# sleep3r/crispy

Hardware: NVIDIA B200
Metric: stream-seconds of 48 kHz audio denoised per wall-second (higher is better)
Workload: dtype f32

## Files before the change

### crispy_b200/csrc/ns_pipe.cuh

```cuda
#pragma once
#include "ns_common.h"
#include "ns_simt.h"

namespace ns {

NS_DEV f4 ld4(const float *p) { return *reinterpret_cast<const f4 *>(p); }

constexpr int kHpThreads = 96;
#ifndef NS_HP_TILE
#define NS_HP_TILE 96
#endif
constexpr int kHpTile = NS_HP_TILE;
constexpr int kHpPitch = kHpTile + 4;
constexpr int kHpStages = 4;
constexpr int kHpAhead = 2;
constexpr int kHpRaw16 = (2 * kHpTile - 8 + 15) / 16 * 16;
static_assert(kFrame % kHpTile == 0 && kHpTile % 8 == 0 && kHpPitch % 32 != 0 && kHpPitch % 4 == 0, "tile geometry");
static_assert(kHpRaw16 % 16 == 0 && kHpRaw16 + 2 * kHpTile <= kHpPitch * 4 && 2 * kHpTile - 8 <= kHpRaw16, "PCM16 staging");
struct HpSmem {
  float tile[kHpStages][32][kHpPitch];
  int landed[kHpStages], done[kHpStages], freed[kHpStages];
};

NS_DEV float load_sample(const Params &p, int stream, long long idx) {
// ... 168 lines not shown
        float v[kHist / 32];
#pragma unroll
        for (int i = 0; i < kHist / 32; i++) v[i] = src[lane + 32 * i];
#pragma unroll
        for (int i = 0; i < kHist / 32; i++) dst[lane + 32 * i] = v[i];
      }
    }
  }
}

#ifndef NS_HP_PAR
#define NS_HP_PAR 1
#endif
constexpr int kHpSeg = 4;
constexpr int kHpSegLen = kHpTile / kHpSeg;
constexpr int kHpYStages = 2;
constexpr int kHpParThreads = 256;
constexpr int kHpParAhead = 1;
static_assert(kHpTile % (4 * kHpSeg) == 0, "segments are whole 16-byte groups");
#ifdef NS_HOST_EMU
inline long long g_hp_respeculated = 0;
#define NS_HP_COUNT_RESPEC() __atomic_add_fetch(&::ns::g_hp_respeculated, 1, __ATOMIC_RELAXED)
#else
#define NS_HP_COUNT_RESPEC() ((void)0)
#endif
#if defined(NS_HP_CLOCKS) && defined(__CUDACC__) && !defined(NS_HOST_EMU)
#define NS_HP_T0() const long long hp_t0_ = clock64()
#define NS_HP_ACC(var) var += clock64() - hp_t0_
#else
#define NS_HP_T0() ((void)0)
#define NS_HP_ACC(var) ((void)0)
#endif
struct HpParSmem {
  HpSmem x;
  float y[kHpYStages][32][kHpPitch];
  float spec[2][kHpSeg + 1][32][2];
  float exact[2][kHpSeg][32][2];
  alignas(16) int bad[2][32][kHpSeg];
  int go;
  int ver;
  int ydone;
  int yfreed;
};

NS_DEV float hp_fast_err(float a, float b, float s) {
  const float ea = b - (s - a), eb = a - (s - b);
  return fabsf(a) >= fabsf(b) ? ea : eb;
}

NS_DEV void highpass_par_body(const Params &p, HpParSmem &sm) {
  const int tid = Simt::tid();
  const int lane = tid & 31, warp = tid >> 5;
  const int s0 = Simt::cta() * 32;
  const int nrows = (p.n_streams - s0) < 32 ? (p.n_streams - s0) : 32;
  const int nsamp = p.n_frames * kFrame;
  const int ntiles = nsamp / kHpTile;
  const bool tail_direct = nsamp >= kHist;
  if (tid < kHpStages) sm.x.landed[tid] = sm.x.done[tid] = sm.x.freed[tid] = 0;
  if (tid == 0) sm.ver = sm.go = sm.ydone = sm.yfreed = 0;
  Simt::cta_sync();
  const long long in0 = (long long)p.frame0 * kFrame;
  const bool in16 = (p.flags & kFlagInI16) != 0;
  const int amask = in16 ? 7 : 3;
  const bool fast = (p.in_stride & amask) == 0 && (in0 & amask) == 0 && (reinterpret_cast<uintptr_t>(p.in) & 15) == 0;
  const bool raw16 = fast && in16;
  const float scale = ((p.flags & kFlagUnitScale) && !in16) ? 32768.0f : 1.0f;
  const bool valid = lane < nrows;
  float m0 = 0.f, m1 = 0.f;
  long long t_work = 0, t_wait = 0, t_wait2 = 0;
  (void)t_work, (void)t_wait, (void)t_wait2;
  const long long t_begin = 0;
  (void)t_begin;
  const double na0 = -(double)-1.99599f, na1 = -(double)0.99600f;
  auto exact_run = [&](const float *xrow, float *yrow, int n4) {
#pragma unroll 2
    for (int c = 0; c < 4 * n4; c += 4) {
      const f4 xv = ld4(xrow + c);
      const float x[4] = {xv.x * scale, xv.y * scale, xv.z * scale, xv.w * scale};
      float y[4];
#pragma unroll
      for (int i = 0; i < 4; i++) {
        const float xi = x[i];
        const float yi = xi + m0;
        const double xd = (double)xi, yd = (double)yi;
        m0 = (float)((double)m1 + fma(na0, yd, -2.0 * xd));
        m1 = (float)fma(na1, yd, xd);
        y[i] = yi;
      }
      *reinterpret_cast<f4 *>(yrow + c) = f4{y[0], y[1], y[2], y[3]};
    }
  };
  if (warp == 1) {
    for (int n = 0; n < ntiles + kHpParAhead; n++) {
      if (n < ntiles) {
        if (n >= kHpStages) {
          NS_HP_T0();
          Simt::flag_wait(&sm.x.freed[n % kHpStages], n - kHpStages + 1, true);
          NS_HP_ACC(t_wait);
        }
        hp_fetch_tile(p, sm.x, s0, nrows, in0, n, fast, lane);
      }
      Simt::cp_async_commit();
      if (n >= kHpParAhead) {
        Simt::cp_async_wait<kHpParAhead>();
        if (raw16) {
          Simt::warp_sync();
          if (lane < nrows) {
            float *row = sm.x.tile[(n - kHpParAhead) % kHpStages][lane];
#pragma unroll 4
            for (int c = 0; c < kHpTile; c += 4) {
              const uint32_t *rw = reinterpret_cast<const uint32_t *>(reinterpret_cast<const char *>(row) + kHpRaw16 + 2 * c);
              const uint32_t r0 = rw[0], r1 = rw[1];
              *reinterpret_cast<f4 *>(row + c) = f4{(float)(int16_t)(r0 & 0xFFFFu), (float)(int16_t)(r0 >> 16),
                                                    (float)(int16_t)(r1 & 0xFFFFu), (float)(int16_t)(r1 >> 16)};
            }
          }
        }
        Simt::fence_cta();
        Simt::warp_sync();
        if (lane == 0) Simt::flag_set(&sm.x.landed[(n - kHpParAhead) % kHpStages], n - kHpParAhead + 1);
      }
    }
  } else if (warp == 0) {
    float *st = p.state + (long long)(s0 + (valid ? lane : 0)) * kStateFloats;
    if (valid) m0 = st[kStHp], m1 = st[kStHp + 1];
    const float a0f = 1.99599f, na1f = -0.99600f;
    auto spec_tile = [&](int n) {
      const float *row = sm.x.tile[n % kHpStages][lane];
      float(*rec)[32][2] = sm.spec[n & 1];
      for (int v = 0; v < kHpSeg; v++) {
        rec[v][lane][0] = m0, rec[v][lane][1] = m1;
#pragma unroll 2
        for (int c = v * kHpSegLen; c < (v + 1) * kHpSegLen; c += 4) {
          const f4 xv = ld4(row + c);
          const float x[4] = {xv.x * scale, xv.y * scale, xv.z * scale, xv.w * scale};
#pragma unroll
          for (int i = 0; i < 4; i++) {
            const float xi = x[i];
            const float yi = xi + m0;
            const float ph = a0f * yi, pl = fmaf(a0f, yi, -ph);
            const float b = -2.0f * xi;
            const float ch = fmaf(-2.0f, xi, m1), cl = hp_fast_err(m1, b, ch);
            const float s1 = ch + ph;
            const float e1 = hp_fast_err(ch, ph, s1);
            m0 = s1 + ((cl + pl) + e1);
            m1 = fmaf(na1f, yi, xi);
          }
        }
      }
      rec[kHpSeg][lane][0] = m0, rec[kHpSeg][lane][1] = m1;
    };
    auto settle = [&](int k, bool next_speculated) {
      Simt::flag_poll(&sm.ver, kHpSeg * (k + 1), false);
      Simt::fence_cta();
      if (valid) {
        static_assert(kHpSeg == 4, "one 16-byte load fetches a lane's four flags");
        struct alignas(16) I4 {
          int x, y, z, w;
        };
        const I4 bd = *reinterpret_cast<const I4 *>(sm.bad[k & 1][lane]);
        const int v0 = bd.x ? 0 : bd.y ? 1 : bd.z ? 2 : bd.w ? 3 : -1;
        if (v0 >= 0) {
          NS_HP_COUNT_RESPEC();
          m0 = sm.exact[k & 1][v0][lane][0], m1 = sm.exact[k & 1][v0][lane][1];
          const int c0 = (v0 + 1) * kHpSegLen;
          exact_run(sm.x.tile[k % kHpStages][lane] + c0, sm.y[k % kHpYStages][lane] + c0, (kHpTile - c0) / 4);
          if (next_speculated) spec_tile(k + 1);
        }
      }
      Simt::fence_cta();
      Simt::warp_sync();
      if (lane == 0) {
        Simt::flag_store(&sm.ydone, k + 1);
        Simt::flag_store(&sm.x.freed[k % kHpStages], k + 1);
        if (next_speculated) Simt::flag_store(&sm.go, k + 2);
      }
    };
    for (int n = 0; n < ntiles; n++) {
      {
        NS_HP_T0();
        Simt::flag_wait(&sm.x.landed[n % kHpStages], n + 1, false);
        NS_HP_ACC(t_wait);
      }
      {
        NS_HP_T0();
        if (valid) spec_tile(n);
        NS_HP_ACC(t_work);
      }
      if (n >= 1) {
        NS_HP_T0();
        settle(n - 1, true);
        NS_HP_ACC(t_wait2);
      } else {
        Simt::fence_cta();
        Simt::warp_sync();
        if (lane == 0) Simt::flag_store(&sm.go, 1);
      }
    }
    if (ntiles > 0) settle(ntiles - 1, false);
    if (valid) {
      st[kStHp] = m0;
      st[kStHp + 1] = m1;
    }
  } else if (warp == 2) {
    hp_copy_rows(p.state + (long long)s0 * kStateFloats + kStHist, kStateFloats, p.hp + (long long)s0 * p.hp_stride,
                 p.hp_stride, nrows, lane);
    Simt::warp_sync();
    for (int n = 0; n < ntiles; n++) {
      {
        NS_HP_T0();
        Simt::flag_wait(&sm.ydone, n + 1, true);
        NS_HP_ACC(t_wait);
      }
      NS_HP_T0();
      float(*tile)[kHpPitch] = sm.y[n % kHpYStages];
      const int base = n * kHpTile;
      if (lane < kHpTile / 4) {
        const int c = 4 * lane;
        float *dsth = p.hp + (long long)s0 * p.hp_stride + kHist + base + c;
        const int hidx = base + c - (nsamp - kHist);
        if (tail_direct && hidx >= 0) {
          float *dsts = p.state + (long long)s0 * kStateFloats + kStHist + hidx;
          for (int r = 0; r < nrows; r++, dsth += p.hp_stride, dsts += kStateFloats) {
            const f4 v = ld4(&tile[r][c]);
            *reinterpret_cast<f4 *>(dsth) = v;
            *reinterpret_cast<f4 *>(dsts) = v;
          }
        } else {
#pragma unroll 8
          for (int r = 0; r < nrows; r++, dsth += p.hp_stride) *reinterpret_cast<f4 *>(dsth) = ld4(&tile[r][c]);
        }
      }
      Simt::warp_sync();
      NS_HP_ACC(t_work);
      if (lane == 0) Simt::flag_set(&sm.yfreed, n + 1);
    }
    if (!tail_direct) {
      Simt::fence_cta();
      Simt::warp_sync();
      for (int r = 0; r < nrows; r++) {
        const float *src = p.hp + (long long)(s0 + r) * p.hp_stride + nsamp;
        float *dst = p.state + (long long)(s0 + r) * kStateFloats + kStHist;
        float v[kHist / 32];
#pragma unroll
        for (int i = 0; i < kHist / 32; i++) v[i] = src[lane + 32 * i];
#pragma unroll
        for (int i = 0; i < kHist / 32; i++) dst[lane + 32 * i] = v[i];
      }
    }
  } else if (warp != 4) {
    const int v = warp == 3 ? 0 : warp - 4;
    for (int n = 0; n < ntiles; n++) {
      {
        NS_HP_T0();
        Simt::flag_wait(&sm.go, n + 1, true);
        NS_HP_ACC(t_wait);
      }
      if (n >= kHpYStages) {
        NS_HP_T0();
        Simt::flag_wait(&sm.yfreed, n - kHpYStages + 1, true);
        NS_HP_ACC(t_wait2);
      }
      NS_HP_T0();
      if (valid) {
        m0 = sm.spec[n & 1][v][lane][0], m1 = sm.spec[n & 1][v][lane][1];
        exact_run(sm.x.tile[n % kHpStages][lane] + v * kHpSegLen, sm.y[n % kHpYStages][lane] + v * kHpSegLen, kHpSegLen / 4);
        sm.exact[n & 1][v][lane][0] = m0, sm.exact[n & 1][v][lane][1] = m1;
        sm.bad[n & 1][lane][v] =
            (f2u(m0) != f2u(sm.spec[n & 1][v + 1][lane][0])) | (f2u(m1) != f2u(sm.spec[n & 1][v + 1][lane][1]));
      }
      Simt::fence_cta();
      Simt::warp_sync();
      NS_HP_ACC(t_work);
      if (lane == 0) Simt::atomic_add_shared(&sm.ver, 1);
    }
  }
#if defined(NS_HP_CLOCKS) && defined(__CUDACC__) && !defined(NS_HOST_EMU)
  if (Simt::cta() == 0 && lane == 0 && warp != 4)
    printf("K0 warp %d: %d tiles, work %lld, wait %lld, wait2 %lld cycles\n", warp, ntiles, t_work, t_wait, t_wait2);
#endif
}

template <int R>
struct PitchSmem {
  static constexpr int kHLen = R * kFrame + 1248;
  static constexpr int kXlpFloats = (R * kLpStride > kHLen) ? R * kLpStride : kHLen;
  alignas(16) float xr[R * kLpStride];
  alignas(16) float xlp[kXlpFloats];
  alignas(16) float ac[R][8];
  alignas(16) float lpc2[R][8];
  alignas(16) float fx[R][12];
  alignas(16) int fi[R][12];
  alignas(16) float xx[R];
  alignas(16) float s10[R][12];
#ifdef NS_PITCH_PAD_BYTES
  char pad[NS_PITCH_PAD_BYTES];
#endif
  int best0[R], best1[R], T0[R], nk[R];
  int n_tri[4], n_sgl[4];
  union {
    struct {
      alignas(16) float xc[R][152];
      alignas(16) float sb6[R][148];
    };
    struct {
      uint32_t tri[4][R * 16], sgl[4][R * 16];
      alignas(16) float dots[R][64];
    };
  };
};

struct Best2 {
  float n0, d0, n1, d1;
  int p0, p1;
};
NS_DEV void best_init(Best2 &b) {
  b.n0 = b.n1 = -1.f;
  b.d0 = b.d1 = 0.f;
  b.p0 = 0;
  b.p1 = 1;
}
NS_DEV void best_insert(Best2 &b, float num, float syy, int i) {
  if (num * b.d1 > b.n1 * syy) {
    if (num * b.d0 > b.n0 * syy) {
      b.n1 = b.n0;
      b.d1 = b.d0;
      b.p1 = b.p0;
      b.n0 = num;
      b.d0 = syy;
      b.p0 = i;
    } else {
      b.n1 = num;
      b.d1 = syy;
      b.p1 = i;
    }
  }
}

NS_DEV void best_insert_sel(Best2 &b, bool valid, float num, float syy, int i) {
  const bool c1 = valid && (num * b.d1 > b.n1 * syy);
  const bool c0 = c1 && (num * b.d0 > b.n0 * syy);
  b.n1 = c0 ? b.n0 : (c1 ? num : b.n1);
  b.d1 = c0 ? b.d0 : (c1 ? syy : b.d1);
  b.p1 = c0 ? b.p0 : (c1 ? i : b.p1);
  b.n0 = c0 ? num : b.n0;
  b.d0 = c0 ? syy : b.d0;
  b.p0 = c0 ? i : b.p0;
}

constexpr int kDotXy0 = 62;
NS_DEV int rd_T1(int k, int T0) { return (2 * T0 + k) / (2 * k); }
NS_DEV int rd_T1b(int k, int T0, int T1) {
  if (k == 2) return (T1 + T0 > 384) ? T0 : T0 + T1;
  const int sc = (k == 6 || k == 12) ? 5 : ((k & 1) ? 2 : 3);
  return (2 * sc * T0 + k) / (2 * k);
}
NS_DEV float pitch_gain_f(float xy, float xx, float yy) { return xy / sqrtf(1.f + xx * yy); }

#ifndef NS_DOT_UNROLL
#define NS_DOT_UNROLL 4
#endif
#define NS_PRAGMA(x) _Pragma(#x)
#define NS_UNROLL(n) NS_PRAGMA(unroll n)
template <bool D4>
struct Acc4 {
  float s = 0.f;
  NS_DEV void add(int, float v) { s += v; }
  NS_DEV float sum() const { return s; }
};
template <>
struct Acc4<true> {
  float s[4] = {0.f, 0.f, 0.f, 0.f};
  NS_DEV void add(int t, float v) { s[t] += v; }
  NS_DEV float sum() const { return ((s[0] + s[1]) + s[2]) + s[3]; }
};
template <int SP>
constexpr bool kSpDot4 = SP >= 1;
template <int SP>
constexpr bool kSpDot4Xcorr = SP >= 2;

template <int N, bool D4 = false>
NS_DEV float dot_shifted(const float *x, const float *yrow, int yoff) {
  static_assert(N % 4 == 0, "whole float4s");
  const float *ya = yrow + (yoff & ~3);
  const bool p1 = (yoff & 1) != 0, p2 = (yoff & 2) != 0;
  f4 lo = ld4(ya), hi = ld4(ya + 4), xv = ld4(x);
  Acc4<D4> sum;
  NS_UNROLL(NS_DOT_UNROLL)
  for (int j = 0; j < N; j += 4) {
    const f4 hi_n = ld4(ya + j + 8), xv_n = ld4(x + j + 4);
    const float a0 = p1 ? lo.y : lo.x, a1 = p1 ? lo.z : lo.y, a2 = p1 ? lo.w : lo.z, a3 = p1 ? hi.x : lo.w,
                a4 = p1 ? hi.y : hi.x, a5 = p1 ? hi.z : hi.y;
    const float y0 = p2 ? a2 : a0, y1 = p2 ? a3 : a1, y2 = p2 ? a4 : a2, y3 = p2 ? a5 : a3;
    sum.add(0, xv.x * y0);
    sum.add(1, xv.y * y1);
    sum.add(2, xv.z * y2);
    sum.add(3, xv.w * y3);
    lo = hi;
    hi = hi_n;
    xv = xv_n;
  }
  return sum.sum();
}
template <int N, int S, bool D4 = false>
NS_DEV float dot_fixed_shift(const float *x, const float *ya) {
  f4 lo = ld4(ya), hi = ld4(ya + 4), xv = ld4(x);
  Acc4<D4> sum;
  NS_UNROLL(NS_DOT_UNROLL)
  for (int j = 0; j < N; j += 4) {
    const f4 hi_n = ld4(ya + j + 8), xv_n = ld4(x + j + 4);
    const float w[8] = {lo.x, lo.y, lo.z, lo.w, hi.x, hi.y, hi.z, hi.w};
    sum.add(0, xv.x * w[S]);
    sum.add(1, xv.y * w[S + 1]);
    sum.add(2, xv.z * w[S + 2]);
    sum.add(3, xv.w * w[S + 3]);
    lo = hi;
    hi = hi_n;
    xv = xv_n;
  }
  return sum.sum();
}
template <int N, int S>
NS_DEV void dot3_fixed_shift(const float *x, const float *ya, float &s0, float &s1, float &s2) {
  f4 w0 = ld4(ya), w1 = ld4(ya + 4), w2 = ld4(ya + 8), xv = ld4(x);
  float a0 = 0.f, a1 = 0.f, a2 = 0.f;
  NS_UNROLL(NS_DOT_UNROLL)
  for (int j = 0; j < N; j += 4) {
    const f4 w2_n = ld4(ya + j + 12), xv_n = ld4(x + j + 4);
    const float w[12] = {w0.x, w0.y, w0.z, w0.w, w1.x, w1.y, w1.z, w1.w, w2.x, w2.y, w2.z, w2.w};
    a0 += xv.x * w[S];
    a1 += xv.x * w[S + 1];
    a2 += xv.x * w[S + 2];
    a0 += xv.y * w[S + 1];
    a1 += xv.y * w[S + 2];
    a2 += xv.y * w[S + 3];
    a0 += xv.z * w[S + 2];
    a1 += xv.z * w[S + 3];
    a2 += xv.z * w[S + 4];
    a0 += xv.w * w[S + 3];
    a1 += xv.w * w[S + 4];
    a2 += xv.w * w[S + 5];
    w0 = w1;
    w1 = w2;
    w2 = w2_n;
    xv = xv_n;
  }
  s0 = a0;
  s1 = a1;
  s2 = a2;
}
template <int N, bool D4 = false>
NS_DEV void dot3_shifted(const float *x, const float *yrow, int yoff, float &s0, float &s1, float &s2) {
  const float *ya = yrow + (yoff & ~3);
  const bool p1 = (yoff & 1) != 0, p2 = (yoff & 2) != 0;
  f4 w0 = ld4(ya), w1 = ld4(ya + 4), w2 = ld4(ya + 8), xv = ld4(x);
  Acc4<D4> a2, a1, a0;
  NS_UNROLL(NS_DOT_UNROLL)
  for (int j = 0; j < N; j += 4) {
    const f4 w2_n = ld4(ya + j + 12), xv_n = ld4(x + j + 4);
    const float b0 = p1 ? w0.y : w0.x, b1 = p1 ? w0.z : w0.y, b2 = p1 ? w0.w : w0.z, b3 = p1 ? w1.x : w0.w,
                b4 = p1 ? w1.y : w1.x, b5 = p1 ? w1.z : w1.y, b6 = p1 ? w1.w : w1.z, b7 = p1 ? w2.x : w1.w;
    const float y0 = p2 ? b2 : b0, y1 = p2 ? b3 : b1, y2 = p2 ? b4 : b2, y3 = p2 ? b5 : b3, y4 = p2 ? b6 : b4,
                y5 = p2 ? b7 : b5;
    a0.add(0, xv.x * y0);
    a1.add(0, xv.x * y1);
    a2.add(0, xv.x * y2);
    a0.add(1, xv.y * y1);
    a1.add(1, xv.y * y2);
    a2.add(1, xv.y * y3);
    a0.add(2, xv.z * y2);
    a1.add(2, xv.z * y3);
    a2.add(2, xv.z * y4);
    a0.add(3, xv.w * y3);
    a1.add(3, xv.w * y4);
    a2.add(3, xv.w * y5);
    w0 = w1;
    w1 = w2;
    w2 = w2_n;
    xv = xv_n;
  }
  s0 = a0.sum();
  s1 = a1.sum();
  s2 = a2.sum();
}
template <bool D4 = false>
NS_DEV float dot480_shifted(const float *row, int yoff) { return dot_shifted<480, D4>(row + 384, row, yoff); }

NS_DEV void syy_recurrence(float syy, const float *y, int len, int n, float *out) {
  for (int i0 = 0; i0 < n; i0 += 4) {
    const f4 ya = ld4(y + i0 + len), yb = ld4(y + i0);
    const float d0 = ya.x * ya.x - yb.x * yb.x, d1 = ya.y * ya.y - yb.y * yb.y, d2 = ya.z * ya.z - yb.z * yb.z,
                d3 = ya.w * ya.w - yb.w * yb.w;
    f4 o;
    o.x = syy;
    syy += d0;
    syy = syy < 1.f ? 1.f : syy;
    o.y = syy;
    syy += d1;
    syy = syy < 1.f ? 1.f : syy;
    o.z = syy;
    syy += d2;
    syy = syy < 1.f ? 1.f : syy;
    o.w = syy;
    syy += d3;
    syy = syy < 1.f ? 1.f : syy;
    *reinterpret_cast<f4 *>(out + i0) = o;
  }
}

template <int N>
NS_DEV float sumsq_from(float acc, const float *y) {
  static_assert(N % 4 == 0, "whole float4s");
#pragma unroll 4
  for (int j = 0; j < N; j += 4) {
    const f4 v = ld4(y + j);
    acc += v.x * v.x;
    acc += v.y * v.y;
    acc += v.z * v.z;
    acc += v.w * v.w;
  }
  return acc;
}

#if defined(NS_PHASE_CLOCKS) && defined(__CUDACC__) && !defined(NS_HOST_EMU)
__device__ unsigned long long g_pitch_phase_cycles[24];
#define NS_PHASE_BEGIN() long long ns_pc_ = clock64()
#define NS_PHASE_MARK(i)                                                       \
  do {                                                                         \
    if (tid == 0) {                                                            \
      const long long now_ = clock64();                                        \
      atomicAdd(&g_pitch_phase_cycles[i], (unsigned long long)(now_ - ns_pc_)); \
      ns_pc_ = now_;                                                           \
    }                                                                          \
  } while (0)
#else
#define NS_PHASE_BEGIN() do {} while (0)
#define NS_PHASE_MARK(i) do {} while (0)
#endif
template <int R, int NT, int SP = 0>
NS_DEV void pitch_body(const Params &p, PitchSmem<R> &sm) {
  const int tid = Simt::tid();
  NS_PHASE_BEGIN();
  const int runs_per_stream = (p.n_frames + R - 1) / R;
  const int stream = Simt::cta() / runs_per_stream;
  const int t0 = (Simt::cta() % runs_per_stream) * R;
  const int nfr = (p.n_frames - t0) < R ? (p.n_frames - t0) : R;
  const float *row = p.hp + (long long)stream * p.hp_stride + 192 + (long long)t0 * kFrame;
  float *h = sm.xlp;

  if (tid < 4) sm.n_tri[tid] = sm.n_sgl[tid] = 0;
  {
    const int n4 = (nfr * kFrame + 1248) / 4;
    const f4 *src = reinterpret_cast<const f4 *>(row);
    f4 *dst = reinterpret_cast<f4 *>(h);
    for (int i = tid; i < n4; i += NT) dst[i] = src[i];
  }
  Simt::cta_sync();
  NS_PHASE_MARK(1);
  for (int it = tid; it < nfr * (kLpLen / 4); it += NT) {
    const int f = it / (kLpLen / 4), i0 = 4 * (it - f * (kLpLen / 4));
    const float *x = h + f * kFrame + 2 * i0;
    const f4 b4 = ld4(x), c4 = ld4(x + 4);
    f4 v;
    if (i0 == 0)
      v.x = .5f * (.5f * b4.y + b4.x);
    else
      v.x = .5f * (.5f * (x[-1] + b4.y) + b4.x);
    v.y = .5f * (.5f * (b4.y + b4.w) + b4.z);
    v.z = .5f * (.5f * (b4.w + c4.y) + c4.x);
    v.w = .5f * (.5f * (c4.y + c4.w) + c4.z);
    *reinterpret_cast<f4 *>(sm.xr + f * kLpStride + i0) = v;
  }
  Simt::cta_sync();
  NS_PHASE_MARK(2);
  if (R <= 8 && NT >= 64) {
    if (tid < 64) {
      const int l = tid & 31, fl = l / 5, k = l - 5 * fl, f = 4 * (tid >> 5) + fl;
      if (l < 20 && f < nfr) {
        const float *x = sm.xr + f * kLpStride;
        const float *y = x + k;
        f4 xv = ld4(x);
        float y0 = y[0], y1 = y[1], y2 = y[2], y3 = y[3];
        Acc4<kSpDot4Xcorr<SP>> sum;
        NS_UNROLL(NS_DOT_UNROLL)
        for (int i = 0; i < kLpLen - 4; i += 4) {
          const f4 xn = ld4(x + i + 4);
          const float n0 = y[i + 4], n1 = y[i + 5], n2 = y[i + 6], n3 = y[i + 7];
          sum.add(0, xv.x * y0);
          sum.add(1, xv.y * y1);
          sum.add(2, xv.z * y2);
          sum.add(3, xv.w * y3);
          xv = xn;
          y0 = n0, y1 = n1, y2 = n2, y3 = n3;
        }
        float d = 0.f;
        for (int i = k + kLpLen - 4; i < kLpLen; i++) d += x[i] * x[i - k];
        sm.ac[f][k] = sum.sum() + d;
      }
    }
  } else if (NT >= 5 * 32 && R <= 32) {
    const int k = tid >> 5, f = tid & 31;
    if (k < 5 && f < nfr) {
      const float *x = sm.xr + f * kLpStride;
      float sum;
      switch (k) {
        case 0: sum = dot_fixed_shift<kLpLen - 4, 0, kSpDot4Xcorr<SP>>(x, x); break;
        case 1: sum = dot_fixed_shift<kLpLen - 4, 1, kSpDot4Xcorr<SP>>(x, x); break;
        case 2: sum = dot_fixed_shift<kLpLen - 4, 2, kSpDot4Xcorr<SP>>(x, x); break;
        case 3: sum = dot_fixed_shift<kLpLen - 4, 3, kSpDot4Xcorr<SP>>(x, x); break;
        default: sum = dot_fixed_shift<kLpLen - 4, 0, kSpDot4Xcorr<SP>>(x, x + 4); break;
      }
      float d = 0.f;
      for (int i = k + kLpLen - 4; i < kLpLen; i++) d += x[i] * x[i - k];
      sm.ac[f][k] = sum + d;
    }
  } else {
    for (int it = tid; it < nfr * 5; it += NT) {
      const int f = it / 5, k = it - f * 5;
      const float *x = sm.xr + f * kLpStride;
      const float sum = dot_shifted<kLpLen - 4, kSpDot4Xcorr<SP>>(x, x, k);
      float d = 0.f;
      for (int i = k + kLpLen - 4; i < kLpLen; i++) d += x[i] * x[i - k];
      sm.ac[f][k] = sum + d;
    }
  }
  Simt::cta_sync();
  NS_PHASE_MARK(3);
  if (tid < nfr) {
    const int f = tid;
    float ac[5], lpc[4] = {0.f, 0.f, 0.f, 0.f};
#pragma unroll
    for (int k = 0; k < 5; k++) ac[k] = sm.ac[f][k];
    ac[0] *= 1.0001f;
#pragma unroll
    for (int i = 1; i <= 4; i++) ac[i] -= ac[i] * (.008f * i) * (.008f * i);
    float error = ac[0];
    if (ac[0] != 0.f) {
      for (int i = 0; i < 4; i++) {
        float rr = 0.f;
        for (int j = 0; j < i; j++) rr += lpc[j] * ac[i - j];
        rr += ac[i + 1];
        const float r = -rr / error;
        lpc[i] = r;
        for (int j = 0; j < ((i + 1) >> 1); j++) {
          const float t1 = lpc[j], t2 = lpc[i - 1 - j];
          lpc[j] = t1 + r * t2;
          lpc[i - 1 - j] = t2 + r * t1;
        }
        error = error - r * r * error;
        if (error < .001f * ac[0]) break;
      }
    }
    float tmp = 1.f;
#pragma unroll
    for (int i = 0; i < 4; i++) {
      tmp = .9f * tmp;
      lpc[i] = lpc[i] * tmp;
    }
    sm.lpc2[f][0] = lpc[0] + .8f;
    sm.lpc2[f][1] = lpc[1] + .8f * lpc[0];
    sm.lpc2[f][2] = lpc[2] + .8f * lpc[1];
    sm.lpc2[f][3] = lpc[3] + .8f * lpc[2];
    sm.lpc2[f][4] = .8f * lpc[3];
  }
  Simt::cta_sync();
  NS_PHASE_MARK(4);
  for (int it = tid; it < nfr * (kLpLen / 4); it += NT) {
    const int f = it / (kLpLen / 4), i0 = 4 * (it - f * (kLpLen / 4));
    const float *x = sm.xr + f * kLpStride + i0;
    const float *n = sm.lpc2[f];
    const f4 z4 = f4{0.f, 0.f, 0.f, 0.f};
    const f4 p4 = (i0 >= 8) ? ld4(x - 8) : z4, q4 = (i0 >= 4) ? ld4(x - 4) : z4, r4 = ld4(x);
    const float w[9] = {p4.w, q4.x, q4.y, q4.z, q4.w, r4.x, r4.y, r4.z, r4.w};
    const float n0 = n[0], n1 = n[1], n2 = n[2], n3 = n[3], n4 = n[4];
    float o[4];
#pragma unroll
    for (int u = 0; u < 4; u++) {
      float sum = w[5 + u];
      sum += n0 * w[4 + u];
      sum += n1 * w[3 + u];
      sum += n2 * w[2 + u];
      sum += n3 * w[1 + u];
      sum += n4 * w[u];
      o[u] = sum;
    }
    *reinterpret_cast<f4 *>(sm.xlp + f * kLpStride + i0) = f4{o[0], o[1], o[2], o[3]};
  }
  Simt::cta_sync();
  NS_PHASE_MARK(5);
  for (int it = tid; it < nfr * 440; it += NT) {
    const int f = it / 440, m = it - f * 440;
    sm.xr[f * kLpStride + m] = (m < 432) ? sm.xlp[f * kLpStride + 2 * m] : 0.f;
  }
  Simt::cta_sync();
  NS_PHASE_MARK(6);
  constexpr int NW = NT / 32;
  static_assert(NW >= 4, "chain warps B and C, the coarse helper and at least one worker warp");
  const int chain_lane = tid & 31;
  const bool chain_b = (tid >> 5) == NW - 2 && chain_lane < nfr, chain_c = (tid >> 5) == NW - 3 && chain_lane < nfr;
  float ch_acc = chain_b ? 1.f : 0.f;
  float ch_p1 = 0.f, ch_p2 = 0.f, ch_p3 = 0.f;
  int ch_blk = 0;
  auto chain_run = [&](int budget, bool recur_b) {
    if (!chain_b && !chain_c) return;
    const int f = chain_lane;
    const float *y = sm.xlp + f * kLpStride + (chain_c ? 384 : 0);
    for (; budget > 0 && ch_blk < 30; budget--, ch_blk++) {
      const float *q = y + 16 * ch_blk;
      const f4 v0 = ld4(q), v1 = ld4(q + 4), v2 = ld4(q + 8), v3 = ld4(q + 12);
      if constexpr (kSpDot4<SP>) {
        if (chain_c) {
          ch_acc += v0.x * v0.x, ch_p1 += v0.y * v0.y, ch_p2 += v0.z * v0.z, ch_p3 += v0.w * v0.w;
          ch_acc += v1.x * v1.x, ch_p1 += v1.y * v1.y, ch_p2 += v1.z * v1.z, ch_p3 += v1.w * v1.w;
          ch_acc += v2.x * v2.x, ch_p1 += v2.y * v2.y, ch_p2 += v2.z * v2.z, ch_p3 += v2.w * v2.w;
          ch_acc += v3.x * v3.x, ch_p1 += v3.y * v3.y, ch_p2 += v3.z * v3.z, ch_p3 += v3.w * v3.w;
          if (ch_blk == 29) ch_acc = ((ch_acc + ch_p1) + ch_p2) + ch_p3;
        }
      }
      if (!kSpDot4<SP> || !chain_c) {
        ch_acc += v0.x * v0.x, ch_acc += v0.y * v0.y, ch_acc += v0.z * v0.z, ch_acc += v0.w * v0.w;
        ch_acc += v1.x * v1.x, ch_acc += v1.y * v1.y, ch_acc += v1.z * v1.z, ch_acc += v1.w * v1.w;
        ch_acc += v2.x * v2.x, ch_acc += v2.y * v2.y, ch_acc += v2.z * v2.z, ch_acc += v2.w * v2.w;
        ch_acc += v3.x * v3.x, ch_acc += v3.y * v3.y, ch_acc += v3.z * v3.z, ch_acc += v3.w * v3.w;
      }
      if (ch_blk == 29 && chain_c) {
        sm.xx[f] = ch_acc;
        sm.xr[f * kLpStride + 432] = ch_acc;
      }
    }
    if (chain_b) {
      if (ch_blk < 30 || !recur_b) return;
      const int lo0 = 2 * sm.best0[f] - 2, lo1 = 2 * sm.best1[f] - 2;
      const int r1 = lo0 < lo1 ? lo0 : lo1, r2 = lo0 < lo1 ? lo1 : lo0;
      auto clampi = [](int v) { return v < 0 ? 0 : (v > 294 ? 294 : v); };
      const int a0 = clampi(r1), b0 = clampi(r2 > r1 + 5 ? r2 : r1 + 5), last = clampi(r2 + 5);
      float syy = ch_acc;
      for (int i0 = 0; i0 < last; i0 += 4) {
        const f4 ya = ld4(y + i0 + 480), yb = ld4(y + i0);
        const float d[4] = {ya.x * ya.x - yb.x * yb.x, ya.y * ya.y - yb.y * yb.y, ya.z * ya.z - yb.z * yb.z,
                            ya.w * ya.w - yb.w * yb.w};
#pragma unroll
        for (int u = 0; u < 4; u++) {
          const int i = i0 + u;
          if ((unsigned)(i - a0) < 5u) sm.s10[f][i - a0] = syy;
          if ((unsigned)(i - b0) < 5u) sm.s10[f][5 + i - b0] = syy;
          syy += d[u];
          syy = syy < 1.f ? 1.f : syy;
        }
      }
      ch_blk = 1000;
    } else {
      float *yyl = sm.xr + f * kLpStride + 432;
      for (; budget > 0 && ch_blk < 30 + 24; budget--, ch_blk++) {
        const int i1 = 1 + 16 * (ch_blk - 30);
        float yy = ch_acc;
#pragma unroll
        for (int h = 0; h < 4; h++) {
          const int i0 = i1 + 4 * h;
          const f4 a = ld4(y - i0 - 3), c = ld4(y + 477 - i0);
          const float av[4] = {a.w * a.w, a.z * a.z, a.y * a.y, a.x * a.x};
          const float cv[4] = {c.w * c.w, c.z * c.z, c.y * c.y, c.x * c.x};
#pragma unroll
          for (int u = 0; u < 4; u++) {
            yy = yy + av[u] - cv[u];
            yyl[i0 + u] = yy < 0.f ? 0.f : yy;
          }
        }
        ch_acc = yy;
      }
    }
  };
  if (tid >= NT - 32) {
    const int l = tid - (NT - 32);
    if (l < nfr) {
      const float *y4 = sm.xr + l * kLpStride;
      syy_recurrence(sumsq_from<240>(1.f, y4), y4, 240, 147, sm.sb6[l]);
    }
  }
  constexpr bool kD4x = kSpDot4Xcorr<SP>;
  constexpr int kLpl = kD4x ? 4 : 8, kQpf = 152 / kLpl;
  for (int it = tid; it < nfr * kQpf; it += NT) {
    const int f = it / kQpf, q = it - f * kQpf;
    const float *y4 = sm.xr + f * kLpStride;
    const float *x4 = y4 + 192;
    const float *yb = y4 + kLpl * q;
    Acc4<kD4x> a[kLpl];
    f4 w0 = ld4(yb), w1 = ld4(yb + 4);
#pragma unroll 2
    for (int j = 0; j < 240; j += 4) {
      const f4 xv = ld4(x4 + j), w2 = ld4(yb + j + 8);
      const float w[12] = {w0.x, w0.y, w0.z, w0.w, w1.x, w1.y, w1.z, w1.w, w2.x, w2.y, w2.z, w2.w};
      const float xt[4] = {xv.x, xv.y, xv.z, xv.w};
#pragma unroll
      for (int t = 0; t < 4; t++)
#pragma unroll
        for (int l = 0; l < kLpl; l++) a[l].add(t, xt[t] * w[l + t]);
      w0 = w1;
      w1 = w2;
    }
    float *dst = sm.xc[f] + kLpl * q;
#pragma unroll
    for (int l = 0; l < kLpl; l += 4)
      *reinterpret_cast<f4 *>(dst + l) = f4{a[l].sum(), a[l + 1].sum(), a[l + 2].sum(), a[l + 3].sum()};
  }
  chain_run(25, false);
  Simt::cta_sync();
  NS_PHASE_MARK(7);
  if (NW > R && (tid >> 5) < R) {
    const int f = tid >> 5, lane = tid & 31;
    if (f < nfr) {
      float sc[5], xcv[5], syv[5];
      float t0v = -1.f, t1v = -1.f, t1num = 0.f, t0num = 0.f;
      int nvalid = 0;
#pragma unroll
      for (int u = 0; u < 5; u++) {
        const int i = lane + 32 * u;
        const bool in = i < 147;
        xcv[u] = in ? sm.xc[f][i] : 0.f;
        syv[u] = in ? sm.sb6[f][i] : 1.f;
        const float x16 = xcv[u] * 1e-12f, num = x16 * x16;
        const bool valid = in && xcv[u] > 0.f;
        sc[u] = valid ? num / syv[u] : -1.f;
        nvalid += valid ? 1 : 0;
        const bool a = sc[u] > t0v, bb = sc[u] > t1v;
        t1v = a ? t0v : (bb ? sc[u] : t1v);
        t1num = a ? t0num : (bb ? num : t1num);
        t0v = a ? sc[u] : t0v;
        t0num = a ? num : t0num;
      }
#pragma unroll
      for (int d = 16; d > 0; d >>= 1) {
        const float o0 = Simt::shfl_xor(t0v, d), o1 = Simt::shfl_xor(t1v, d), n0 = Simt::shfl_xor(t0num, d), n1 = Simt::shfl_xor(t1num, d);
        nvalid += Simt::shfl_xor(nvalid, d);
        bool a = o0 > t0v, bb = o0 > t1v;
        t1v = a ? t0v : (bb ? o0 : t1v);
        t1num = a ? t0num : (bb ? n0 : t1num);
        t0v = a ? o0 : t0v;
        t0num = a ? n0 : t0num;
        bb = o1 > t1v;
        t1num = bb ? n1 : t1num;
        t1v = bb ? o1 : t1v;
      }
      const float thr = nvalid >= 2 ? t1v * (1.f - 2e-4f) : -1.f;
      unsigned mine = 0u;
      int cnt = 0;
#pragma unroll
      for (int u = 0; u < 5; u++)
        if (sc[u] >= 0.f && sc[u] >= thr) mine |= 1u << u, cnt++;
      int total = cnt;
#pragma unroll
      for (int d = 16; d > 0; d >>= 1) total += Simt::shfl_xor(total, d);
      Best2 b;
      best_init(b);
      if (total > 32 || (nvalid >= 2 && !(t1num >= 1e-30f))) {
        if (lane == 0) {
          for (int i = 0; i < 147; i++) {
            const float xc = sm.xc[f][i];
            const float x16 = xc * 1e-12f;
            best_insert_sel(b, xc > 0.f, x16 * x16, sm.sb6[f][i], i);
          }
        }
      } else {
        for (int s = 0; s < total; s++) {
          int mn = 0x7FFFFFFF;
#pragma unroll
          for (int u = 0; u < 5; u++)
            if (mine & (1u << u)) {
              const int i = lane + 32 * u;
              mn = i < mn ? i : mn;
            }
#pragma unroll
          for (int d = 16; d > 0; d >>= 1) {
            const int o = Simt::shfl_xor(mn, d);
            mn = o < mn ? o : mn;
          }
          const int src = mn & 31, u = mn >> 5;
          float xc = 0.f, sy = 1.f;
#pragma unroll
          for (int uu = 0; uu < 5; uu++)
            if (uu == u) xc = xcv[uu], sy = syv[uu];
          xc = Simt::shfl(xc, src);
          sy = Simt::shfl(sy, src);
          const float x16 = xc * 1e-12f;
          best_insert_sel(b, xc > 0.f, x16 * x16, sy, mn);
          if (lane == src) mine &= ~(1u << u);
        }
      }
      if (lane == 0) {
        sm.best0[f] = b.p0;
        sm.best1[f] = b.p1;
      }
    }
  } else if (NW <= R && tid < nfr) {
    const int f = tid;
    Best2 b;
    best_init(b);
    for (int i0 = 0; i0 < 147; i0 += 4) {
      const f4 xc4 = ld4(sm.xc[f] + i0), sy4 = ld4(sm.sb6[f] + i0);
      const float xcv[4] = {xc4.x, xc4.y, xc4.z, xc4.w}, syv[4] = {sy4.x, sy4.y, sy4.z, sy4.w};
#pragma unroll
      for (int u = 0; u < 4; u++) {
        if (i0 + u < 147) {
          const float x16 = xcv[u] * 1e-12f;
          best_insert_sel(b, xcv[u] > 0.f, x16 * x16, syv[u], i0 + u);
        }
      }
    }
    sm.best0[f] = b.p0;
    sm.best1[f] = b.p1;
  }
  chain_run(20, false);
  Simt::cta_sync();
  NS_PHASE_MARK(8);
  for (int it = tid; it < nfr * 10; it += NT) {
    const int f = it / 10, c = it - f * 10;
    const float *lp = sm.xlp + f * kLpStride;
    const int c0 = 2 * sm.best0[f], c1 = 2 * sm.best1[f];
    const int i = (c < 5) ? (c0 - 2 + c) : (c1 - 2 + (c - 5));
    const int dd = i - c0;
    const bool ok = (i >= 0) && (i < 294) && (c < 5 || dd > 2 || dd < -2);
    float sum = 0.f;
    if (ok) sum = dot480_shifted<kSpDot4<SP>>(lp, i);
    sm.fi[f][c] = ok ? i : -1;
    sm.fx[f][c] = sum < -1.f ? -1.f : sum;
  }
  chain_run(1000, true);
  Simt::cta_sync();
  NS_PHASE_MARK(9);
  if (tid < nfr) {
    const int f = tid;
    const float *y = sm.xlp + f * kLpStride;
    const int lo0 = 2 * sm.best0[f] - 2, lo1 = 2 * sm.best1[f] - 2;
    auto xcorr_at = [&](int i) -> float {
      const int d0 = i - lo0, d1 = i - lo1;
      if (d0 >= 0 && d0 < 5 && sm.fi[f][d0] == i) return sm.fx[f][d0];
      if (d1 >= 0 && d1 < 5 && sm.fi[f][5 + d1] == i) return sm.fx[f][5 + d1];
      return 0.f;
    };
    Best2 b;
    best_init(b);
    const int r1 = lo0 < lo1 ? lo0 : lo1, r2 = lo0 < lo1 ? lo1 : lo0;
    auto clampi = [](int v) { return v < 0 ? 0 : (v > 294 ? 294 : v); };
    const int a0 = clampi(r1), a1 = clampi(r1 + 5), b0 = clampi(r2 > r1 + 5 ? r2 : r1 + 5), b1 = clampi(r2 + 5);
    auto checked = [&](int from, int to, const float *syy) {
      for (int i = from; i < to; i++) {
        const float xc = xcorr_at(i);
        const float x16 = xc * 1e-12f;
        best_insert_sel(b, xc > 0.f, x16 * x16, syy[i - from], i);
      }
    };
    checked(a0, a1, sm.s10[f]);
    checked(b0, b1, sm.s10[f] + 5);
    const int bp = b.p0;
    int offset = 0;
    if (bp > 0 && bp < 293) {
      const float a = xcorr_at(bp - 1), bb = xcorr_at(bp), cc = xcorr_at(bp + 1);
      if ((cc - a) > .7f * (bb - a))
        offset = 1;
      else if ((a - cc) > .7f * (bb - cc))
        offset = -1;
    }
    const int pitch_index = kPitchMax - (2 * bp - offset);
    int T0 = pitch_index / 2;
    if (T0 >= 384) T0 = 383;
    sm.T0[f] = T0;
  }
  Simt::cta_sync();
  NS_PHASE_MARK(10);
  for (int it = tid; it < nfr * 16; it += NT) {
    const int f = it >> 4, k = it & 15;
    if (k == 0) continue;
    const int T0 = sm.T0[f];
    if (k > 1 && rd_T1(k, T0) < 30) continue;
    if (k == kMaxK || rd_T1(k + 1, T0) < 30) sm.nk[f] = k;
    const int Tc = (k == 1) ? T0 : rd_T1(k, T0);
    {
      const int idx = Simt::atomic_add_shared(&sm.n_tri[0], 1);
      (&sm.tri[0][0])[idx] = (uint32_t)(f | (Tc << 5) | (k << 14));
    }
    if (k > 1) {
      const int T1b = rd_T1b(k, T0, Tc);
      const int idx = Simt::atomic_add_shared(&sm.n_sgl[0], 1);
      (&sm.sgl[0][0])[idx] = (uint32_t)(f | (T1b << 5) | (k << 14));
    }
  }
  Simt::cta_sync();
  NS_PHASE_MARK(11);
  {
    const int w = tid >> 5, lane = tid & 31;
    const int n_tri = sm.n_tri[0], n_sgl = sm.n_sgl[0];
    const int tri_warps = (n_tri + 31) >> 5, sgl_warps = (n_sgl + 31) >> 5;
    for (int job = w; job < tri_warps + sgl_warps; job += NW) {
      if (job < tri_warps) {
        const int it = job * 32 + lane;
        if (it < n_tri) {
          const int e = (&sm.tri[0][0])[it];
          const int f = e & 31, Tc = (e >> 5) & 0x1FF, k = e >> 14;
          const float *row = sm.xlp + f * kLpStride;
          float sp, sc, sm1;
          dot3_shifted<480, kSpDot4<SP>>(row + 384, row, 384 - Tc - 1, sp, sc, sm1);
          const int d = 2 + 4 * (k - 2);
          sm.dots[f][k == 1 ? 0 : d] = sm1;
          sm.dots[f][k == 1 ? kDotXy0 : d + 1] = sc;
          sm.dots[f][k == 1 ? 1 : d + 2] = sp;
        }
      } else {
        const int it = (job - tri_warps) * 32 + lane;
        if (it < n_sgl) {
          const int e = (&sm.sgl[0][0])[it];
          const int f = e & 31, lag = (e >> 5) & 0x1FF, k = e >> 14;
          const float *row = sm.xlp + f * kLpStride;
          sm.dots[f][2 + 4 * (k - 2) + 3] = dot_shifted<480, kSpDot4<SP>>(row + 384, row, 384 - lag);
        }
      }
    }
  }
  Simt::cta_sync();
  NS_PHASE_MARK(12);
  for (int it = tid; it < nfr * 16; it += NT) {
    const int f = it >> 4, k = it & 15;
    uint32_t *tab = p.tab + ((long long)stream * p.chunk_cap + (t0 + f)) * kTabWords;
    const int T0 = sm.T0[f], nk = sm.nk[f];
    if (k == 0) {
      tab[0] = (uint32_t)T0 | ((uint32_t)nk << 16);
      tab[1] = 0u;
      continue;
    }
    if (k > nk) continue;
    const float *yyl = sm.xr + f * kLpStride + 432;
    const float xx = sm.xx[f];
    float xy, yy, c0, c1, c2;
    int T;
    if (k == 1) {
      T = T0;
      xy = sm.dots[f][kDotXy0];
      yy = yyl[T0];
      c0 = sm.dots[f][0];
      c1 = xy;
      c2 = sm.dots[f][1];
    } else {
      const int d = 2 + 4 * (k - 2);
      T = rd_T1(k, T0);
      const int T1b = rd_T1b(k, T0, T);
      c0 = sm.dots[f][d];
      c1 = sm.dots[f][d + 1];
      c2 = sm.dots[f][d + 2];
      xy = .5f * (c1 + sm.dots[f][d + 3]);
      yy = .5f * (yyl[T] + yyl[T1b]);
    }
    const float g = pitch_gain_f(xy, xx, yy);
    const float bxy = xy < 0.f ? 0.f : xy;
    float pg = (yy <= bxy) ? 1.f : bxy / (yy + 1.f);
    if (pg > g) pg = g;
    int offset = 0;
    if ((c2 - c0) > .7f * (c1 - c0))
      offset = 1;
    else if ((c0 - c2) > .7f * (c1 - c2))
      offset = -1;
    int pi = 2 * T + offset;
    if (pi < kPitchMin) pi = kPitchMin;
    uint32_t *e = tab + 2 + 3 * (k - 1);
    e[0] = (uint32_t)T | ((uint32_t)pi << 16);
    e[1] = f2u(g);
    e[2] = f2u(pg);
  }
  NS_PHASE_MARK(13);
}

NS_DEV void pitchscan_body(const Params &p, int warps_per_cta) {
  const int lane = Simt::tid() & 31;
  const int stream = Simt::cta() * warps_per_cta + (Simt::tid() >> 5);
  if (stream >= p.n_streams) return;
  float *st = p.state + (long long)stream * kStateFloats;
  int last_period = reinterpret_cast<int *>(st)[kStLastPeriod];
  float last_gain = st[kStLastGain];
  const uint32_t *tab = p.tab + (long long)stream * p.chunk_cap * kTabWords;
  float *rec = p.rec + (long long)stream * p.chunk_cap * kRecFloats;
  const int k = lane + 1;
  for (int t = 0; t < p.n_frames; t++, tab += kTabWords, rec += kRecFloats) {
    const uint32_t hdr = tab[0];
    const int T0 = (int)(hdr & 0xFFFFu), nk = (int)(hdr >> 16);
    uint32_t w0 = 0u;
    float g1 = 0.f, pg = 0.f;
    if (k <= nk) {
      w0 = tab[2 + 3 * lane];
      g1 = u2f(tab[3 + 3 * lane]);
      pg = u2f(tab[4 + 3 * lane]);
    }
    const float g0 = Simt::shfl(g1, 0);
    const int T1 = (int)(w0 & 0xFFFFu);
    const int prev_period = last_period / 2;
    bool pass = (k == 1);
    if (k >= 2 && k <= nk) {
      const int dT = T1 > prev_period ? T1 - prev_period : prev_period - T1;
      float cont;
      if (dT <= 1)
        cont = last_gain;
      else if (dT <= 2 && 5 * k * k < T0)
        cont = .5f * last_gain;
      else
        cont = 0.f;
      float thresh = .7f * g0 - cont;
      if (thresh < .3f) thresh = .3f;
      if (T1 < 90) {
        thresh = .85f * g0 - cont;
        if (thresh < .4f) thresh = .4f;
      } else if (T1 < 60) {
        thresh = .9f * g0 - cont;
        if (thresh < .5f) thresh = .5f;
      }
      pass = g1 > thresh;
    }
    const unsigned m = Simt::ballot(pass);
    int win = 0;
    for (int b = 14; b > 0; b--)
      if (m & (1u << b)) {
        win = b;
        break;
      }
    const int pi = (int)(Simt::shfl((int)w0, win) >> 16) & 0xFFFF;
    const float gain = Simt::shfl(pg, win);
    last_period = pi;
    last_gain = gain;
    if (lane == 0) {
      reinterpret_cast<int *>(rec)[kRecPitchIndex] = pi;
      rec[kRecPitchGain] = gain;
    }
  }
  if (lane == 0) {
    reinterpret_cast<int *>(st)[kStLastPeriod] = last_period;
    st[kStLastGain] = last_gain;
  }
}

struct SpecTw {
  cf w480[480];
  cf w960[244];
#ifndef NS_FFT3
  cf tw3[64];
#else
  cf tw3[72];
#endif
};
struct Tab {
  const SpecTw *s;
  const Tables *g;
  NS_DEV cf w480(int i) const { return s->w480[i]; }
  NS_DEV cf w960(int i) const { return s->w960[i]; }
#ifndef NS_FFT3
  NS_DEV cf tw3(int r, int k) const { return s->tw3[(r - 1) * 16 + k]; }
#else
  NS_DEV cf tw3(int r, int k) const { return s->tw3[(r - 1) * 8 + k]; }
#endif
  NS_DEV float win(int i) const { return Simt::ldg(g->win + i); }
  NS_DEV float dct(int i) const { return Simt::ldg(g->dct + i); }
  NS_DEV int bin_band(int i) const { return Simt::ldg(g->bin_band + i); }
  NS_DEV int eband(int i) const { return Simt::ldg(g->eband + i); }
  NS_DEV f4 win4(int i) const { return ldg_f4(g->win + i); }
  NS_DEV f4 bin_frac4(int i) const { return ldg_f4(g->bin_frac + i); }
  static NS_DEV f4 ldg_f4(const float *p) {
#if defined(__CUDACC__) && !defined(NS_HOST_EMU)
    const float4 v = Simt::ldg4(p);
    return f4{v.x, v.y, v.z, v.w};
#else
    return *reinterpret_cast<const f4 *>(p);
#endif
  }
};

struct Grp {
  int tid, lane, warp, bar;
};
NS_DEV void gsync(const Grp &g) { Simt::group_sync(g.bar, kGroupThreads); }
NS_DEV cf cmul(cf a, cf b) {
  cf c;
  c.x = fmaf(a.x, b.x, -(a.y * b.y));
  c.y = fmaf(a.x, b.y, a.y * b.x);
  return c;
}
NS_DEV cf cadd(cf a, cf b) { return cf{a.x + b.x, a.y + b.y}; }
NS_DEV cf csub(cf a, cf b) { return cf{a.x - b.x, a.y - b.y}; }
NS_DEV cf mul_neg_i(cf a) { return cf{a.y, -a.x}; }
NS_DEV cf mul_pos_i(cf a) { return cf{-a.y, a.x}; }

template <int R>
struct Dft;
template <>
struct Dft<3> {
  static NS_DEV void run(cf *v) {
    const float s = 0.86602540378443864676f;
    cf a = cadd(v[1], v[2]), b = csub(v[1], v[2]);
    cf m = cf{fmaf(-0.5f, a.x, v[0].x), fmaf(-0.5f, a.y, v[0].y)};
    cf n = cf{s * b.x, s * b.y};
    v[0] = cadd(v[0], a);
    v[1] = cadd(m, mul_neg_i(n));
    v[2] = cadd(m, mul_pos_i(n));
  }
};
template <>
struct Dft<4> {
  static NS_DEV void run(cf *v) {
    cf t0 = cadd(v[0], v[2]), t1 = csub(v[0], v[2]);
    cf t2 = cadd(v[1], v[3]), t3 = mul_neg_i(csub(v[1], v[3]));
    v[0] = cadd(t0, t2);
    v[2] = csub(t0, t2);
    v[1] = cadd(t1, t3);
    v[3] = csub(t1, t3);
  }
};
template <>
struct Dft<5> {
  static NS_DEV void run(cf *v) {
    const float c1 = 0.30901699437494742410f, c2 = -0.80901699437494742410f;
    const float s1 = 0.95105651629515357212f, s2 = 0.58778525229247312917f;
// ... 1215 lines not shown
```

Baseline: 348,700.

## Screen pitch lag candidates with cheap xcorr and recompute exact survivors only

When there are more warps than frames, the coarse pitch cross-correlation now uses a plain FMA accumulator instead of the exact dot4 accumulator. A warp-level screen then bounds each lag's score using an error estimate and keeps only lags that could still be in the top two. Only those survivors (at most 32 per frame, otherwise all 147) are recomputed with the exact dot_shifted routine before best-lag selection. This trades an extra screening pass and a CTA sync for less exact-precision work, and depends on the error bound being conservative enough to keep results bit-identical.

```diff
diff --git a/crispy_b200/csrc/ns_pipe.cuh b/crispy_b200/csrc/ns_pipe.cuh
--- a/crispy_b200/csrc/ns_pipe.cuh
+++ b/crispy_b200/csrc/ns_pipe.cuh
@@ -494,6 +494,8 @@
     struct {
       alignas(16) float xc[R][152];
       alignas(16) float sb6[R][148];
+      int slag[R][32];
+      int scnt[R];
     };
     struct {
       uint32_t tri[4][R * 16], sgl[4][R * 16];
@@ -714,6 +716,94 @@
   return acc;
 }
 
+constexpr float kScreenErr = 6e-5f;
+constexpr int kScreenMaxSurvivors = 32;
+#ifdef NS_P6_STATS
+extern long g_p6_stats[3];
+#endif
+
+NS_DEV int popc32(unsigned v) {
+#if defined(__CUDACC__) && !defined(NS_HOST_EMU)
+  return __popc(v);
+#else
+  return __builtin_popcount(v);
+#endif
+}
+NS_DEV int ctz32(unsigned v) {
+#if defined(__CUDACC__) && !defined(NS_HOST_EMU)
+  return __ffs((int)v) - 1;
+#else
+  return __builtin_ctz(v);
+#endif
+}
+
+NS_DEV int coarse_screen(const float *y4, const float *xc, const float *syy, int *slag, int lane) {
+  const float *x4 = y4 + 192;
+  float sxx = 0.f, e = 0.f;
+  for (int j = 4 * lane; j < 240; j += 128) {
+    const f4 v = ld4(x4 + j);
+    sxx += v.x * v.x, sxx += v.y * v.y, sxx += v.z * v.z, sxx += v.w * v.w;
+  }
+  for (int j = 4 * lane; j < 388; j += 128) {
+    const f4 v = ld4(y4 + j);
+    e += v.x * v.x, e += v.y * v.y, e += v.z * v.z, e += v.w * v.w;
+  }
+#pragma unroll
+  for (int d = 16; d > 0; d >>= 1) {
+    sxx += Simt::shfl_xor(sxx, d);
+    e += Simt::shfl_xor(e, d);
+  }
+  const float dx = kScreenErr * sqrtf(sxx + 1e-38f) * sqrtf(e + 1e-38f) + 1e-38f;
+  bool finite = dx < 3.0e38f;
+  auto bound = [&](int i, bool upper) {
+    const bool in = i < 147;
+    const float xf = in ? xc[i] : 0.f, sy = in ? syy[i] : 1.f;
+    const float xb = upper ? xf + dx : xf - dx, b16 = xb * 1e-12f;
+    return (in && xb > 0.f) ? b16 * b16 / sy * (upper ? 1.f + 1e-6f : 1.f - 1e-6f) : -1.f;
+  };
+  float l0 = -1.f, l1 = -1.f;
+#pragma unroll
+  for (int u = 0; u < 5; u++) {
+    const int i = lane + 32 * u;
+    finite = finite && (i >= 147 || fabsf(xc[i]) < 3.0e38f);
+    const float lo = bound(i, false);
+    l1 = lo > l0 ? l0 : (lo > l1 ? lo : l1);
+    l0 = lo > l0 ? lo : l0;
+  }
+#pragma unroll
+  for (int d = 16; d > 0; d >>= 1) {
+    const float o0 = Simt::shfl_xor(l0, d), o1 = Simt::shfl_xor(l1, d);
+    l1 = o0 > l0 ? l0 : (o0 > l1 ? o0 : l1);
+    l0 = o0 > l0 ? o0 : l0;
+    l1 = o1 > l1 ? o1 : l1;
+  }
+  const float thr = l1 * (1.f - 2e-4f);
+  unsigned word[5];
+  int total = 0;
+#pragma unroll
+  for (int u = 0; u < 5; u++) {
+    word[u] = Simt::ballot(bound(lane + 32 * u, true) >= thr);
+    total += popc32(word[u]);
+  }
+  const bool all_finite = Simt::ballot(!finite) == 0u;
+  if (all_finite && total <= kScreenMaxSurvivors && l1 >= 1e-30f) {
+    int s = lane, lag = -1;
+#pragma unroll
+    for (int u = 0; u < 5; u++) {
+      const int c = popc32(word[u]);
+      if (lag < 0 && s < c) {
+        unsigned w = word[u];
+        for (int k = 0; k < s; k++) w &= w - 1u;
+        lag = 32 * u + ctz32(w);
+      }
+      s -= c;
+    }
+    if (lag >= 0) slag[lane] = lag;
+    return total;
+  }
+  return -1;
+}
+
 #if defined(NS_PHASE_CLOCKS) && defined(__CUDACC__) && !defined(NS_HOST_EMU)
 __device__ unsigned long long g_pitch_phase_cycles[24];
 #define NS_PHASE_BEGIN() long long ns_pc_ = clock64()
@@ -970,13 +1060,14 @@
     }
   }
   constexpr bool kD4x = kSpDot4Xcorr<SP>;
-  constexpr int kLpl = kD4x ? 4 : 8, kQpf = 152 / kLpl;
+  constexpr bool kScreen = NW > R;
+  constexpr int kLpl = (kD4x && !kScreen) ? 4 : 8, kQpf = 152 / kLpl;
   for (int it = tid; it < nfr * kQpf; it += NT) {
     const int f = it / kQpf, q = it - f * kQpf;
     const float *y4 = sm.xr + f * kLpStride;
     const float *x4 = y4 + 192;
     const float *yb = y4 + kLpl * q;
-    Acc4<kD4x> a[kLpl];
+    Acc4<kD4x && !kScreen> a[kLpl];
     f4 w0 = ld4(yb), w1 = ld4(yb + 4);
 #pragma unroll 2
     for (int j = 0; j < 240; j += 4) {
@@ -986,7 +1077,12 @@
 #pragma unroll
       for (int t = 0; t < 4; t++)
 #pragma unroll
-        for (int l = 0; l < kLpl; l++) a[l].add(t, xt[t] * w[l + t]);
+        for (int l = 0; l < kLpl; l++) {
+          if constexpr (kScreen)
+            a[l].s = fmaf(xt[t], w[l + t], a[l].s);
+          else
+            a[l].add(t, xt[t] * w[l + t]);
+        }
       w0 = w1;
       w1 = w2;
     }
@@ -998,6 +1094,42 @@
   chain_run(25, false);
   Simt::cta_sync();
   NS_PHASE_MARK(7);
+  if constexpr (kScreen) {
+    if ((tid >> 5) < nfr) {
+      const int f = tid >> 5, lane = tid & 31;
+      const int survivors = coarse_screen(sm.xr + f * kLpStride, sm.xc[f], sm.sb6[f], sm.slag[f], lane);
+      if (lane == 0) sm.scnt[f] = survivors;
+#ifdef NS_P6_STATS
+      if (lane == 0) {
+        __atomic_fetch_add(&g_p6_stats[survivors >= 0 ? 0 : 1], 1, __ATOMIC_RELAXED);
+        if (survivors >= 0) __atomic_fetch_add(&g_p6_stats[2], survivors, __ATOMIC_RELAXED);
+      }
+#elif defined(NS_PHASE_CLOCKS) && defined(__CUDACC__) && !defined(NS_HOST_EMU)
+      if (lane == 0) {
+        atomicAdd(&g_pitch_phase_cycles[survivors >= 0 ? 16 : 17], 1ull);
+        if (survivors >= 0) atomicAdd(&g_pitch_phase_cycles[18], (unsigned long long)survivors);
+      }
+#endif
+    }
+    Simt::cta_sync();
+    int cnt[R], total = 0;
+#pragma unroll
+    for (int f = 0; f < R; f++) {
+      cnt[f] = f < nfr ? (sm.scnt[f] < 0 ? 147 : sm.scnt[f]) : 0;
+      total += cnt[f];
+    }
+    for (int it = tid; it < total; it += NT) {
+      int f = 0, k = it;
+#pragma unroll
+      for (int g = 0; g < R - 1; g++)
+        if (f == g && k >= cnt[g]) k -= cnt[g], f++;
+      const float *y4 = sm.xr + f * kLpStride;
+      const int lag = sm.scnt[f] < 0 ? k : sm.slag[f][k];
+      sm.xc[f][lag] = dot_shifted<240, kD4x>(y4 + 192, y4, lag);
+    }
+    chain_run(20, false);
+    Simt::cta_sync();
+  }
   if (NW > R && (tid >> 5) < R) {
     const int f = tid >> 5, lane = tid & 31;
     if (f < nfr) {
@@ -1101,7 +1233,7 @@
     sm.best0[f] = b.p0;
     sm.best1[f] = b.p1;
   }
-  chain_run(20, false);
+  if constexpr (!kScreen) chain_run(20, false);
   Simt::cta_sync();
   NS_PHASE_MARK(8);
   for (int it = tid; it < nfr * 10; it += NT) {
```

Measured after the change: 340,500, median of 6. -2.4%, worse.
